# Wumpf/yasph2d

Hardware: AMD Instinct MI355X
Metric: particle-steps/sec (whole node), 2D DFSPH dam-break (higher is better)
Workload: dtype f32

## Files before the change

include/sphx.h:

```cpp
#ifndef SPHX_H
#define SPHX_H

#include <stddef.h>
#include <stdint.h>

#ifdef __cplusplus
extern "C" {
#endif

#define SPHX_ABI_VERSION 5

enum {
    SPHX_OK = 0,
    SPHX_ERR_INVALID_ARGUMENT = 1,
    SPHX_ERR_NO_DEVICE = 2,
    SPHX_ERR_HIP = 3,
    SPHX_ERR_NOT_READY = 4,
    SPHX_ERR_NONFINITE = 5,
    SPHX_ERR_NEIGHBOR_PANIC = 6,
    SPHX_ERR_CAPACITY = 7,
    SPHX_ERR_OUT_OF_DOMAIN = 8
};

enum {
// ... 217 lines not shown
int sphx_gauge_levels(sphx_ctx* ctx, const sphx_gauge* gauges , uint32_t n_gauges, int kernel_kind, int field, float iso,
                      uint32_t flags, sphx_gauge_rec* out , float* values );
int sphx_gauge_reduce(const float* values, const sphx_gauge* gauges, uint32_t n_gauges, float iso, sphx_gauge_rec* out);
int sphx_probe_record(sphx_ctx* ctx, const float* points_xy , uint32_t m_points, const sphx_gauge* gauges ,
                      uint32_t n_gauges, int kernel_kind, int field, float iso, uint32_t max_frames, uint32_t every);
int sphx_probe_get_status(const sphx_ctx* ctx, sphx_probe_status* out);
int sphx_probe_read(sphx_ctx* ctx, uint32_t first_frame, uint32_t n_frames, sphx_probe_rec* points_out ,
                    sphx_gauge_rec* gauges_out , sphx_stats_frame* info );

int sphx_debug_correction_counts(sphx_ctx* ctx, uint64_t out[3]);
int sphx_debug_quiet_counts(sphx_ctx* ctx, uint64_t out[2]);
int sphx_debug_takeover_counts(sphx_ctx* ctx, uint64_t out[3]);

int sphx_debug_rigid_counts(sphx_ctx* ctx, uint64_t out[3]);
int sphx_debug_rigid_predict_counts(sphx_ctx* ctx, uint64_t out[4]);
int sphx_debug_download_accel(sphx_ctx* ctx, float* out_xy);
int sphx_debug_download_wcsph_half_step(sphx_ctx* ctx, float* pos_xy, float* vel_xy, float* density, uint32_t* particle_id);

int sphx_clear_cached(sphx_ctx* ctx);
int sphx_step_begin(sphx_ctx* ctx, float dt_prev, float* out_vmax);
int sphx_step_finish(sphx_ctx* ctx, float dt, sphx_step_stats* out_stats);

typedef struct sphx_timer_law {
    uint32_t adaptive;
    float cfl_factor;
    float particle_diameter;
    uint32_t reserved;
    uint64_t timestep_min_ns;
    uint64_t timestep_max_ns;
    uint64_t simulation_step_ns;
// ... 374 lines not shown
```

yasph2d_amd/__init__.py:

```python
import ctypes as C

import numpy as np

from . import _lib
from ._lib import (FLAG_DENSITY_ITER_CAP, FLAG_DIVERGENCE_ITER_CAP, FLAG_DENSE_CELL, FLAG_NEIGHBOR_CAP, FLAG_STRAY_PARTICLES, FLAG_WARMUP, KERNEL_POLY6,
                   KERNEL_SPIKY, KERNEL_WENDLAND_C2, VISCOSITY_PHYSICAL, VISCOSITY_XSPH, SphxError, SphxKernelTime, SphxParams, SphxStepStats)

__all__ = ["SphxContext", "FluidParticleWorld", "TimeManager", "DFSPHSolver", "DFSPHMultiSolver", "default_params", "duration_from_secs_f32",
           "duration_as_secs_f32", "SphxError", "WCSPHSolver", "VISCOSITY_XSPH", "VISCOSITY_PHYSICAL", "SAMPLE_FIELDS", "gauge_elevation", "contour_chain", "contour_lines", "contour_merge",
           "sample_merge", "query_merge", "render_fit", "render_merge", "track_merge", "track_merge_frames", "write_png", "SCENE_RECT", "TRACK_FIELDS", "MULTI_TRACK_FIELDS", "FIELD_NAMES", "STATS_DTYPE", "STATS_FRAME_DTYPE",
           "GAUGE_DTYPE", "GAUGE_REC_DTYPE", "PROBE_REC_DTYPE", "gauge_reduce"]


def _p(a):
    return a.ctypes.data_as(C.c_void_p) if a is not None else None


LISTS_32BIT = 0xFFFFFFFF


_VISCOSITY_MODELS = {"xsph": VISCOSITY_XSPH, "physical": VISCOSITY_PHYSICAL}


def default_params(smoothing_factor=2.0, particle_density=10000.0, fluid_density=100.0, device=0, fixed_iterations=(0, 0), viscosity="xsph",
# ... 807 lines not shown
        return int(out[0]), int(out[1])

    def takeover_counts(self):
        out = (C.c_uint64 * 3)()
        self._chk(self.L.sphx_debug_takeover_counts(self.h, out))
        return int(out[0]), int(out[1]), int(out[2])

    def rigid_counts(self):
        out = (C.c_uint64 * 3)()
        self._chk(self.L.sphx_debug_rigid_counts(self.h, out))
        return int(out[0]), int(out[1]), int(out[2])

    def rigid_predict_counts(self):
        out = (C.c_uint64 * 4)()
        self._chk(self.L.sphx_debug_rigid_predict_counts(self.h, out))
        return int(out[0]), int(out[1]), int(out[2]), int(out[3])

    def download_accel(self):
        out = np.zeros((self.n, 2), np.float32)
        self._chk(self.L.sphx_debug_download_accel(self.h, out.ctypes.data_as(C.c_void_p)))
        return out

    def download_wcsph_half_step(self):
        n = self.n
        out = dict(pos=np.zeros((n, 2), np.float32), vel=np.zeros((n, 2), np.float32), density=np.zeros(n, np.float32), ids=np.zeros(n, np.uint32))
        self._chk(self.L.sphx_debug_download_wcsph_half_step(self.h, _p(out["pos"]), _p(out["vel"]), _p(out["density"]), _p(out["ids"])))
        return out

    def grid_info(self, which=0):
        out = (C.c_uint32 * 4)()
# ... 695 lines not shown
```

yasph2d_amd/_lib.py:

```python
import ctypes as C
import os
import subprocess

_HERE = os.path.dirname(os.path.abspath(__file__))
LIB_PATH = os.environ.get("SPHX_LIB") or os.path.join(_HERE, "libsphx.so")
CSRC = os.path.join(_HERE, "csrc")

OK, ERR_INVALID_ARGUMENT, ERR_NO_DEVICE, ERR_HIP, ERR_NOT_READY, ERR_NONFINITE, ERR_NEIGHBOR_PANIC, ERR_CAPACITY, ERR_OUT_OF_DOMAIN = range(9)
FLAG_NEIGHBOR_CAP, FLAG_DENSITY_ITER_CAP, FLAG_DIVERGENCE_ITER_CAP, FLAG_WARMUP, FLAG_STRAY_PARTICLES, FLAG_DENSE_CELL = 1, 2, 4, 8, 16, 32
KERNEL_WENDLAND_C2, KERNEL_POLY6, KERNEL_SPIKY = 0, 1, 2
VISCOSITY_XSPH, VISCOSITY_PHYSICAL = 0, 1


class SphxParams(C.Structure):
    _fields_ = [
        ("smoothing_length", C.c_float),
        ("particle_mass", C.c_float),
        ("fluid_density", C.c_float),
        ("particle_radius", C.c_float),
        ("gravity", C.c_float * 2),
        ("grid_min", C.c_float * 2),
        ("xsph_epsilon", C.c_float),
        ("max_avg_density_error", C.c_float),
        ("max_density_iterations", C.c_uint32),
# ... 325 lines not shown
    "sphx_multi_state_load": (_i, [_vp, C.POINTER(_vp), C.POINTER(_u64), _u32, _u32]),
    "sphx_multi_state_digest": (_i, [_vp, C.POINTER(_u64)]),
    "sphx_multi_state_save_file": (_i, [_vp, C.c_char_p]),
    "sphx_multi_state_load_file": (_i, [_vp, C.c_char_p]),
    "sphx_multi_append": (_i, [_vp, _vp, _vp, _u32, C.POINTER(_u32)]),
    "sphx_multi_remove": (_i, [_vp, C.POINTER(SphxRect), _u32, _u32, C.POINTER(_u64)]),
    "sphx_tile_remove_mark": (_i, [_vp, C.POINTER(SphxRect), _u32, _u32]),
    "sphx_tile_remove_fetch": (_i, [_vp, C.POINTER(_u32)]),
    "sphx_tile_append": (_i, [_vp, _vp, _vp, _vp, _u32]),
    "sphx_tile_grow": (_i, [_vp, _u32]),
    "sphx_debug_correction_counts": (_i, [_vp, _vp]),
    "sphx_debug_quiet_counts": (_i, [_vp, _vp]),
    "sphx_debug_takeover_counts": (_i, [_vp, _vp]),
    "sphx_debug_rigid_counts": (_i, [_vp, _vp]),
    "sphx_debug_rigid_predict_counts": (_i, [_vp, _vp]),
    "sphx_debug_download_accel": (_i, [_vp, _vp]),
    "sphx_debug_download_wcsph_half_step": (_i, [_vp, _vp, _vp, _vp, _vp]),
    "sphx_download_by_id": (_i, [_vp, _u32, _u32, _u32, C.POINTER(SphxTrackOut), C.POINTER(_u32)]),
    "sphx_download": (_i, [_vp, _vp, _vp, _vp, _vp]),
    "sphx_download_boundary": (_i, [_vp, _vp, _vp]),
    "sphx_num_particles": (_u32, [_vp]),
    "sphx_num_boundary": (_u32, [_vp]),
    "sphx_sample_points": (_i, [_vp, _vp, _u32, _i, _u32, C.POINTER(SphxSampleOut)]),
    "sphx_sample_grid": (_i, [_vp, _f, _f, _f, _f, _u32, _u32, _i, _u32, C.POINTER(SphxSampleOut)]),
    "sphx_surface_contour": (_i, [_vp, _f, _f, _f, _f, _u32, _u32, _i, _i, _f, _u32, _u32, C.POINTER(SphxContourOut)]),
    "sphx_contour_chain": (_i, [_vp, _u32, _vp, _vp, _vp, C.POINTER(_u32)]),
    "sphx_multi_sample_points": (_i, [_vp, _vp, _u32, _i, _u32, C.POINTER(SphxMultiSampleOut)]),
    "sphx_multi_sample_grid": (_i, [_vp, _f, _f, _f, _f, _u32, _u32, _i, _u32, C.POINTER(SphxMultiSampleOut)]),
    "sphx_sample_merge": (_i, [_u32, C.POINTER(SphxMultiSampleOut), _u32, C.POINTER(SphxMultiSampleOut)]),
    "sphx_multi_query_radius": (_i, [_vp, _vp, _u32, _f, _u64, _u32, C.POINTER(SphxMultiQueryOut)]),
# ... 185 lines not shown
```

yasph2d_amd/csrc/sphx_compute_error_body.inc:

```
    static_assert(!TAKE || KNZ, "the take-over producers are the ones that leave flags");
    constexpr bool SPEC = TAKE && !DIVERGENCE;
    if (la.enabled && la.iter > 1u && scal->loop_done != 0u) return;
    if (dt_dev) dt = *dt_dev;
    if (clear_hist) {
        const uint32_t per = (clear_len + gridDim.x - 1u) / gridDim.x;
        const uint32_t c0 = blockIdx.x * per, c1 = min(c0 + per, clear_len);
        for (uint32_t k = c0 + threadIdx.x; k < c1; k += 256u) clear_hist[k] = 0u;
    }
    __shared__ Stage<2, 0> rec;
    auto put = [&](uint32_t slot, const float4& r) { rec.put_vec01(slot, r); };
    auto take = [&](uint32_t o) { return rec.vec01(o); };
    const uint32_t blk = xcd_bid(K.rev, K.xcd_shift);
    const uint32_t i = blk * 256 + threadIdx.x;
    [[maybe_unused]] bool k_a = false;
    if constexpr (RIGID != 0) {
        static_assert(!DIVERGENCE && PREDICT && KNZ && TAKE, "the rigid form is the density loop's take-over producer with the prediction");
        uint32_t vb = 0;
        if (pa.va.enabled && threadIdx.x < STRIPES) vb = scal->vstripe[threadIdx.x].vmax[pa.va.vslot & 3u];
        const uint32_t verdict = scal->verdict.accel_uniform;
        const float2 v0 = PV.vel[0];
        const uint32_t last = n ? n - 1u : 0u, ic = min(i, last);
        const uint32_t craw = nb.counts[ic];
        const uint32_t wi = (uint32_t)__builtin_amdgcn_readfirstlane(i >> 6);
        const uint32_t ww = wi * 64u < n ? nb.wave[wi] : 0u;
// ... 2 lines not shown
        __shared__ float dt_r;
        if (pa.va.enabled && threadIdx.x < 64) {
            const uint32_t b = wave_max_u32(vb);
            const unsigned long long ns = timer_law_step_ns(pa.law, sqrtf(__uint_as_float(b)));
            const float d = duration_as_secs_f32(ns);
            if (threadIdx.x == 0) dt_r = d;
            if (blockIdx.x == 0) vmax_publish(scal, pa.va, b, pa.law, ns, d);
        }
        if (pa.va.enabled) {
            __syncthreads();
            dt = dt_r;
        }
        k_a = verdict == ta.accel_tag;
        const float4 pvi = make_float4(p_i.x, p_i.y, v0.x + K.ax * dt, v0.y + K.ay * dt);
        const bool finite = ((__float_as_uint(pvi.z) & 0x7f800000u) != 0x7f800000u) && ((__float_as_uint(pvi.w) & 0x7f800000u) != 0x7f800000u);
        DirAhead ahead_r{0xFFFFFFFFu, EMPTY};
        if constexpr (RIGID == 2) {
            if (ta.hist && i < n) {
                uint32_t cx0, cy0;
                cell_of(K, p_i, cx0, cy0);
                ahead_r = dir_ahead(ta.g, cx0, cy0);
            }
        }
        const uint32_t c = i < n ? craw : 0u;
        const bool reaches_static = (c & 0x7fu) != ((c >> 7) & 0x7fu) || (ww >> 31) != 0u;
        const bool walks = __syncthreads_or(reaches_static ? 1 : 0) != 0 || !k_a || !finite || RIGID != 2;
        if (ta.count && threadIdx.x == 0) {
            Stripe& s = scal->stripe[blockIdx.x % STRIPES];
            if (k_a && blk * 256u < n) atomicAdd(walks ? &s.rp_walk : &s.rp_exit, 1u);
            if (!k_a && blockIdx.x == 0) atomicAdd(&s.rp_noverdict, 1u);
// ... 121 lines not shown
```

yasph2d_amd/csrc/sphx_correct_body.inc:

```
    static_assert(!ZS || (!WARM && !TILE), "the skip belongs to the plain corrections");
    static_assert(!QF || ZS, "the decide-first form falls back to the skip's decision");
    float dt = WARM ? ca.dt : (la.enabled ? la.dt : ca.dt);
    if (dt_dev) {
        dt = *dt_dev;
        inv_dt = 1.0f / dt;
    }
    constexpr bool RES = !WARM;
    const bool need_verdict = RES && ra.enabled && (THIN ? vblk == 0u : blockIdx.x == 0);
    const bool judge = need_verdict && threadIdx.x < 64;
    unsigned long long hi = 0, lo = 0, snap_h = 0, snap_l = 0;
    uint32_t sticky = 0;
    uint32_t jmark = ~ra.rseq;
    const uint32_t rp = ra.rseq & 1u;
    if (RES && ra.enabled) {
        const uint32_t done_before = (la.enabled && la.iter > 1u) ? scal->loop_done : 0u;
        if (judge) {
            residual_stripe_load(scal, hi, lo);
            if constexpr (ZS)
                if (threadIdx.x < STRIPES) jmark = scal->mstripe[threadIdx.x].knz_mark;
            snap_h = scal->snap_hi[rp ^ 1u];
            snap_l = scal->snap_lo[rp ^ 1u];
            sticky = scal->flags;
        }
        if (done_before != 0u && done_before < la.iter) {
// ... 111 lines not shown
            __syncthreads();
            if constexpr (THIN && INV_DT) {
                if (!quiet_s && ca.hist && vblk == 0u && threadIdx.x == 0) scal->spec.flags = 0u;
            }
            if (quiet_s) {
                if (zs.count && threadIdx.x == 0) {
                    unsigned long long stands_for = 1ull;
                    if constexpr (THIN) {
                        stands_for = 0ull;
                        for (uint32_t v = vblk; v < vgrid; v += gridDim.x) stands_for += xcd_map(v, vgrid, K.rev, K.xcd_shift) * 256u < n ? 1ull : 0ull;
                    }
                    atomicAdd(&scal->stripe[blockIdx.x % STRIPES].zs_skipped, stands_for);
                    atomicAdd(&scal->stripe[blockIdx.x % STRIPES].zs_quiet, stands_for);
                }
                if constexpr (THIN && INV_DT) {
                    if (ca.hist && vblk == 0u && threadIdx.x == 0) {
                        const uint32_t f = scal->spec.flags;
                        if (f) {
                            atomicOr(&scal->flags, f);
                            scal->spec.flags = 0u;
                        }
                    }
                }
                verdict();
                if constexpr (THIN) SPHX_CORRECT_LEAVE(true);
                float2 pnew = make_float2(0.0f, 0.0f);
                DirAhead ahead{0xFFFFFFFFu, EMPTY};
                if (i < n) {
                    if (INV_DT) {
                        if (ca.hist) {
// ... 180 lines not shown
```

yasph2d_amd/csrc/sphx_handoff.hpp:

```cpp
#pragma once
#include <cstdint>
#include <cstring>

namespace sphx {

struct BuildHandoff {
    enum Kind : uint8_t { None, WarmApplied, FirstErrors };
    Kind kind = None;
    bool has_flags = false, warm_taken = false;
    uint32_t mark_tag = 0;
    struct Taken {
        bool fused, flags_usable, warm_taken;
    };
    static BuildHandoff warm_applied() { return BuildHandoff{WarmApplied, false, false, 0u}; }
    static BuildHandoff first_errors(bool flags, uint32_t tag, bool taken) { return BuildHandoff{FirstErrors, flags, flags && taken, tag}; }
    void clear() { *this = BuildHandoff{}; }
    bool first_errors_pending() const { return kind == FirstErrors; }
    bool take_warm() {
        const bool applied = kind == WarmApplied;
        if (applied) clear();
        return applied;
    }
    Taken take_first_errors(bool first_divergence, uint32_t rseq) {
        if (kind != FirstErrors || !first_divergence) return Taken{false, false, false};
// ... 76 lines not shown
    void filled() { *this = AccelUniform{}; }
    Taken read() {
        const Taken t{owed, false, tag};
        owed = false;
        return t;
    }
    Taken take(bool substitute) {
        const bool k_a = substitute && uniform;
        const Taken t{owed && !k_a, k_a, tag};
        if (t.fill) owed = false;
        uniform = false;
        return t;
    }
};

}
```

yasph2d_amd/csrc/sphx_internal.hpp:

```cpp
#pragma once
#include <hip/hip_runtime.h>

#include <dlfcn.h>

#include <algorithm>
#include <cstdint>
#include <cstdlib>
#include <cstdio>
#include <cstring>
#include <functional>
#include <map>
#include <string>
#include <vector>

#include "../../include/sphx.h"
#include "sphx_handoff.hpp"

namespace sphx {

constexpr uint32_t EMPTY = 0xFFFFFFFFu;
constexpr uint32_t MAX_NEIGHBORS = 64;
constexpr uint32_t BLOCK_SHIFT = 6;
constexpr uint32_t BLOCK_CELLS = 4096;
constexpr uint32_t SCAN_TILE = 4096;
// ... 109 lines not shown
    uint32_t knz_mark;
    uint32_t vmix_mark;
    uint32_t pad[30];
};
static_assert(sizeof(MarkStripe) == 128, "one stripe, one cache line");
struct alignas(128) SpecLine {
    uint32_t flags;
    uint32_t pad0;
    unsigned long long moved;
    uint32_t pad[28];
};
struct alignas(128) VerdictLine {
    uint32_t accel_uniform;
    uint32_t pad[31];
};
struct DevScalars {
    uint32_t flags;
    uint32_t ticket;
    uint32_t sort_total;
    float dt;
    uint32_t loop_done;
    uint32_t pad0;
    unsigned long long snap_hi[2], snap_lo[2];
    uint32_t rigid_exits, rigid_marked;
    uint32_t pad[16];
    Stripe stripe[STRIPES];
    VmaxStripe vstripe[STRIPES];
    MarkStripe mstripe[STRIPES];
    SpecLine spec;
    VerdictLine verdict;
};

struct Mailbox {
    volatile uint32_t seq;
    uint32_t flags;
    uint32_t vmax_sq_bits;
    uint32_t quiet_seq;
    double err_sum;
    unsigned long long nb_entries;
    unsigned long long owned_cum;
    unsigned long long rem_entries;
    uint32_t sort_total;
    uint32_t dt_bits;
    unsigned long long dt_ns;
    volatile uint32_t loop_gen_done;
// ... 185 lines not shown
    uint32_t thin_grid = 0;
    int quiet_takeover_density = 1;
    bool take_over(bool divergence) const {
        return !tile_mode && (divergence || quiet_takeover_density) && (quiet_takeover == 2 || (quiet_takeover == 1 && quiet_hint[divergence ? 1 : 0]));
    }
    unsigned long long thin_launches = 0, takeover_producers = 0;
    int rigid_skip = -1;
    bool rigid_on() const { return !tile_mode && (rigid_skip < 0 ? N >= 4000000u : rigid_skip != 0); }
    sphx::VelMarks velmarks;
    uint32_t gather_seq = 0;
    bool rigid_hint = false;
    uint32_t rigid_judged = 0;
    void rigid_forget() {
        velmarks.wrote();
        accel_uniform.velocities_written();
        rigid_hint = false;
        rigid_judged = 0;
    }
    unsigned long long rigid_launches = 0;
    int rigid_predict = 2;
    sphx::AccelUniform accel_uniform;
    unsigned long long rigid_predict_launches = 0;
    float2* accel = nullptr;
    float *density = nullptr, *alpha = nullptr, *alpha2 = nullptr, *kappa = nullptr, *stiff = nullptr;
    float *kappa2 = nullptr, *stiff2 = nullptr;
    uint32_t *pid = nullptr, *pid2 = nullptr;
    uint32_t *key = nullptr, *order = nullptr;
    uint32_t idx_cap = 0;
    uint32_t soff() const { return capN; }
    float2 *bpos = nullptr, *bpos2 = nullptr;
    uint32_t *bid = nullptr, *bid2 = nullptr;
    sphx::Grid gdyn, gstat;
    bool have_fluid_bbox = false;
    uint32_t fb[4] = {0, 0, 0, 0};
    uint32_t builds_since_cover = 0;
    bool need_expand = false;
    bool need_recover = false;
// ... 97 lines not shown
```

yasph2d_amd/csrc/sphx_kernels.hip:

```cpp
#include "sphx_internal.hpp"
#include "sphx_sqrt.hpp"
#include "sphx_xcd.hpp"

namespace sphx {

__device__ __forceinline__ uint32_t part1by1(uint32_t x) {
    x &= 0xffffu;
    x = (x ^ (x << 8)) & 0x00ff00ffu;
    x = (x ^ (x << 4)) & 0x0f0f0f0fu;
    x = (x ^ (x << 2)) & 0x33333333u;
    x = (x ^ (x << 1)) & 0x55555555u;
    return x;
}
__device__ __forceinline__ uint32_t morton2(uint32_t x, uint32_t y) { return (part1by1(y) << 1) | part1by1(x); }

__device__ __forceinline__ uint32_t spread6(uint32_t v) {
    v &= 63u;
    v = (v | (v << 4)) & 0x30Fu;
    v = (v | (v << 2)) & 0x333u;
    v = (v | (v << 1)) & 0x555u;
    return v;
}
__device__ __forceinline__ uint32_t sat_u16(float v) {
    v = fminf(fmaxf(v, 0.0f), 65535.0f);
// ... 584 lines not shown
    float* r2_out;
    const float* r3_in;
    float* r3_out;
    const uint32_t* u_in;
    uint32_t* u_out;
    DevScalars* count_owned;
    DevScalars* flags;
    float advect_dt;
    uint32_t advect_below;
    uint32_t fix_owner;
    float cell_inv, gmin_x, gmin_y;
    TileRect own;
    uint32_t rank_by_id;
    uint32_t nt_cold;
    uint32_t vmix_tag;
};
#ifndef SPHX_GATHER_PER_LANE
#define SPHX_GATHER_PER_LANE 1
#endif
constexpr uint32_t GATHER_PER_LANE = SPHX_GATHER_PER_LANE;
__global__ __launch_bounds__(256) void k_rank_gather(const uint32_t* __restrict__ order, const uint32_t* __restrict__ cidx, uint32_t n,
                                                      uint32_t n_in, const uint2* __restrict__ fine, GatherArgs a,
                                                      const uint32_t* __restrict__ n_dev, uint32_t rev) {
    if (n_dev) n = min(n, *n_dev);
    const uint32_t b0 = xcd_bid(xcd_packed_rev(rev), xcd_packed_shift(rev)) * (256u * GATHER_PER_LANE);
    if (b0 >= n) return;
    uint2 vref = make_uint2(0u, 0u);
    if (a.vmix_tag) vref = *(const uint2*)a.vel_in;
    bool vmix = false;
    constexpr int RANK_L = 5, RANK_R = 6;
    constexpr uint32_t ORD_HALO = 8, SPAN = 256u * GATHER_PER_LANE;
    static_assert(RANK_L <= (int)ORD_HALO && RANK_R <= (int)ORD_HALO, "window of order[] words in LDS");
    __shared__ uint32_t sord[SPAN + 2 * ORD_HALO];
    uint32_t own[GATHER_PER_LANE];
#pragma unroll
    for (uint32_t u = 0; u < GATHER_PER_LANE; ++u) {
        own[u] = order[min(b0 + u * 256u + threadIdx.x, n - 1u)];
        sord[ORD_HALO + u * 256u + threadIdx.x] = own[u];
    }
    if (threadIdx.x < 2 * ORD_HALO) {
        const int32_t k = threadIdx.x < ORD_HALO ? (int32_t)(b0 + threadIdx.x) - (int32_t)ORD_HALO : (int32_t)(b0 + SPAN + threadIdx.x - ORD_HALO);
        sord[threadIdx.x < ORD_HALO ? threadIdx.x : SPAN + threadIdx.x] = order[(uint32_t)min(max(k, 0), (int32_t)n - 1)];
    }
    bool ok[GATHER_PER_LANE];
    float2 q[GATHER_PER_LANE], v[GATHER_PER_LANE];
    float r1[GATHER_PER_LANE], r2[GATHER_PER_LANE], r3[GATHER_PER_LANE];
    uint32_t id[GATHER_PER_LANE];
#pragma unroll
    for (uint32_t u = 0; u < GATHER_PER_LANE; ++u) {
        const uint32_t i = own[u] & ORDER_INDEX;
        ok[u] = b0 + u * 256u + threadIdx.x < n && i < n_in;
        const uint32_t ic = ok[u] ? i : 0u;
        q[u] = a.pos_in[ic];
        v[u] = a.vel_in ? a.vel_in[ic] : make_float2(0.0f, 0.0f);
        r1[u] = a.r_in ? a.r_in[ic] : 0.0f, r2[u] = a.r2_in ? a.r2_in[ic] : 0.0f, r3[u] = a.r3_in ? a.r3_in[ic] : 0.0f;
        id[u] = a.u_in ? a.u_in[ic] : 0u;
    }
    __syncthreads();
#pragma unroll
    for (uint32_t u = 0; u < GATHER_PER_LANE; ++u) {
        if (!ok[u]) continue;
        const uint32_t p = b0 + u * 256u + threadIdx.x, i = own[u] & ORDER_INDEX;
        uint32_t near[RANK_L + RANK_R + 1];
#pragma unroll
        for (int d = -RANK_L; d <= RANK_R; ++d) near[d + RANK_L] = sord[(int)(ORD_HALO + u * 256u + threadIdx.x) + d];
        uint32_t heads_l = 0, heads_r = 0;
#pragma unroll
        for (int d = 0; d <= RANK_L; ++d) heads_l |= (near[RANK_L - d] >> 31) << d;
#pragma unroll
// ... 56 lines not shown
        if (a.r3_in) a.r3_out[dst] = r3[u];
        if (a.u_in) {
            uint32_t idd = id[u];
            if (a.fix_owner && i < a.advect_below) {
                const uint32_t cx = sat_u16((qd.x - a.gmin_x) * a.cell_inv), cy = sat_u16((qd.y - a.gmin_y) * a.cell_inv);
                if (!rect_has(a.own, cx, cy, 0u)) idd &= 0x7FFFFFFFu;
            }
            store_cold(&a.u_out[dst], idd, a.nt_cold);
            if (a.count_owned) {
                const unsigned long long m = __ballot((idd >> 31) != 0);
                if (m && (threadIdx.x & 63) == (uint32_t)(__ffsll((long long)__ballot(1)) - 1))
                    atomicAdd(&a.count_owned->stripe[blockIdx.x % STRIPES].owned, (unsigned long long)__popcll(m));
            }
        }
    }
    if (a.vmix_tag) {
        const bool ref_bad = (vref.x & 0x7f800000u) == 0x7f800000u || (vref.y & 0x7f800000u) == 0x7f800000u;
        const unsigned long long m = __ballot(vmix || ref_bad);
        if (m && (threadIdx.x & 63) == (uint32_t)(__ffsll((long long)__ballot(1)) - 1)) a.flags->mstripe[blockIdx.x % STRIPES].vmix_mark = a.vmix_tag;
    }
}

__global__ __launch_bounds__(256) void k_iota(uint32_t* __restrict__ a, uint32_t n) {
    const uint32_t i = blockIdx.x * 256 + threadIdx.x;
    if (i < n) a[i] = i;
}
__global__ __launch_bounds__(256) void k_fill_f32(float* __restrict__ a, uint32_t from, uint32_t n, float v) {
    const uint32_t i = from + blockIdx.x * 256 + threadIdx.x;
    if (i < n) a[i] = v;
}
// ... 1369 lines not shown
template <bool DIVERGENCE, bool PREDICT = false, bool KNZ = false, bool TAKE = false>
__global__ TRAV_BOUNDS void k_compute_error(PVr PV, const float* __restrict__ density,
                                                        const float* __restrict__ alpha, uint32_t n, uint32_t soff, Consts K, float dt,
                                                        NbView nb, float* __restrict__ kbuf, float* __restrict__ warm_zero,
                                                        DevScalars* __restrict__ scal, const float* __restrict__ dt_dev, LoopArgs la,
                                                        uint32_t* __restrict__ clear_hist, uint32_t clear_len, PredArgs pa,
                                                        uint32_t* __restrict__ knz, uint32_t knz_tag,
                                                        std::conditional_t<TAKE && !DIVERGENCE, CountArgs, NoTake> ta) {
    constexpr int RIGID = 0;
#include "sphx_compute_error_body.inc"
}

struct RigidTake : CountArgs {
    uint32_t accel_tag;
    uint32_t count;
};
template <bool EXIT>
__global__ TRAV_BOUNDS void k_compute_error_rigid(PVr PV, const float* __restrict__ density,
                                                              const float* __restrict__ alpha, uint32_t n, uint32_t soff, Consts K, float dt,
                                                              NbView nb, float* __restrict__ kbuf, float* __restrict__ warm_zero,
                                                              DevScalars* __restrict__ scal, const float* __restrict__ dt_dev, LoopArgs la,
                                                              uint32_t* __restrict__ clear_hist, uint32_t clear_len, PredArgs pa,
                                                              uint32_t* __restrict__ knz, uint32_t knz_tag, RigidTake ta) {
    constexpr bool DIVERGENCE = false, PREDICT = true, KNZ = true, TAKE = true;
    constexpr int RIGID = EXIT ? 2 : 1;
#include "sphx_compute_error_body.inc"
}

__global__ __launch_bounds__(256) void k_accel_materialize(float2* __restrict__ accel, uint32_t n, uint32_t vgrid, float ax, float ay,
                                                           const DevScalars* __restrict__ scal, uint32_t tag) {
// ... 132 lines not shown
```

yasph2d_amd/csrc/sphx_launch.inc:

```
#include <algorithm>
#include <cmath>

using namespace sphx;

static std::string g_create_error;

#define SPHX_HIP(ctx, expr)                                                        \
    do {                                                                           \
        hipError_t e__ = (expr);                                                   \
        if (e__ != hipSuccess) return (ctx)->fail(SPHX_ERR_HIP, #expr, hipGetErrorString(e__)); \
    } while (0)

namespace {

inline uint32_t nblocks(uint32_t n, uint32_t per = 256) {
    const uint32_t b = (n + per - 1) / per;
    return per == 256 ? (b + 7u) & ~7u : b;
}
inline double kbar_of(const sphx_ctx* c) { return (c->N && c->nb_last) ? (double)c->nb_last / (double)c->N : 12.0; }
inline double list_bytes(const sphx_ctx* c) {
    if (!c->K.remote_cap) return 2.0 + 4.0 * kbar_of(c);
    const double rbar = c->N ? (double)c->rem_last / (double)c->N : 0.5;
    return 2.0 + 4.0 / 64.0 + (4.0 / 3.0) * kbar_of(c) + 4.0 * rbar + 4.0 / 256.0;
}
// ... 492 lines not shown
    c->ahead.valid = false;
    flush_pending_advect(c);
}

int build_grid(sphx_ctx* c, Grid& g, const float2* pos, uint32_t n, const GatherArgs& ga, float advect_dt, bool ring, uint32_t* tile_n = nullptr,
               bool mark_velocities = false) {
    hipStream_t st = c->stream;
    DevScalars* ds = c->d_scal;
    const uint32_t len = g.len();
    const uint32_t nt = nblocks(len, c->scan_two_pass ? SCAN_TILE : SCAN1_TILE);
    const bool counted = &g == &c->gdyn && advect_dt > 0 && !tile_n && c->pending.is_for(n);
    const bool partial = &g == &c->gdyn && tile_n && advect_dt == 0.0f && !counted && c->pending.is_for_first_of(n);
    const uint32_t first = partial ? c->pending.n() : 0u;
    if (&g == &c->gdyn) c->velmarks.wrote();
    if (&g == &c->gdyn) c->accel_uniform.velocities_written();
    if (counted || partial)
        c->pending.forget();
    else
        drop_fused_count(c);
    if (n > first && !counted) {
        const uint32_t gbc = std::max(1u, nblocks(n - first));
        if (advect_dt > 0)
            launch(c, "advect+cell_count", (16.0 + 4 + 4) * n, [&] {
                hipLaunchKernelGGL(k_key_count<true>, dim3(gbc), dim3(256), 0, st, c->pv(), (const float2*)nullptr, n, advect_dt, c->K,
                                   g.view(), g.hist, c->key, ring ? 1u : 0u, ds, first);
            });
        else
            launch(c, "cell_count", (8.0 + 4 + 4) * (n - first), [&] {
                hipLaunchKernelGGL(k_key_count<false>, dim3(gbc), dim3(256), 0, st, PVr{nullptr, nullptr}, pos, n, 0.0f, c->K, g.view(),
                                   g.hist, c->key, ring ? 1u : 0u, ds, first);
// ... 30 lines not shown
                *tile_n = seq;
            }
        }
        const uint32_t gb2 = std::max(8u, (nblocks(ng, 256 * GATHER_PER_LANE) + 7u) & ~7u);
        double gbytes = 4;
        gbytes += ga.vel_in ? (16 + 16) : 16;
        if (ga.r_in) gbytes += 8;
        if (ga.r2_in) gbytes += 8;
        if (ga.r3_in) gbytes += 8;
        if (ga.u_in) gbytes += 8;
        GatherArgs gm = ga;
        if (mark_velocities && &g == &c->gdyn && !tile_n && ga.vel_in) {
            if (++c->gather_seq == 0) c->gather_seq = 1;
            gm.vmix_tag = c->gather_seq;
        }
        if (ng)
            launch(c, "gather_attributes", gbytes * ng, [&] {
                hipLaunchKernelGGL(k_rank_gather, dim3(gb2), dim3(256), 0, st, (const uint32_t*)c->order, (const uint32_t*)c->key, ng, n,
                                   (const uint2*)g.fine, gm, tile_n ? (const uint32_t*)&ds->sort_total : (const uint32_t*)nullptr, xcd_pack(c->K.rev, xcd_shift_of(c)));
            });
        if (ng && gm.vmix_tag) c->velmarks.made(gm.vmix_tag);
    }
    return SPHX_OK;
}

int ensure_index_scratch(sphx_ctx* c) {
    const uint32_t need = std::max(std::max(std::max(c->N, c->capN), c->B), 1u);
    if (need <= c->idx_cap) return SPHX_OK;
    int rc;
    if ((rc = dev_alloc(c, &c->key, need))) return rc;
// ... 225 lines not shown
    if (c->N) {
        const uint32_t n = c->N;
        auto go = [&](auto kernel, const DivArgs& dv) {
            hipLaunchKernelGGL(kernel, dim3(nblocks(n)), dim3(256), 0, st, (const float2*)c->posA, n, c->soff(), c->K, c->gdyn.nview(), c->gstat.nview(),
                               c->nb_list, c->nb_counts, c->nb_wave, c->nb_remote, c->density, c->alpha, c->d_scal, n_dev, dv);
        };
        c->handoff.clear();
        if (fuse && fuse_warm) {
            DivArgs dv{};
            dv.velw = c->vel;
            dv.warm = c->stiff;
            dv.lim = -0.5f * c->K.rho0 * c->K.rho0;
            launch(c, "neighbor_build+density_alpha+divergence_warmstart", (8.0 + list_bytes(c) + 8.0 + 8.0 + 8.0 + 4.0) * n, [&] { go(k_neighbor_build<3>, dv); });
            c->handoff = BuildHandoff::warm_applied();
            c->velmarks.wrote();
            c->accel_uniform.velocities_written();
        } else if (fuse && fuse_div) {
            DivArgs dv{};
            dv.vel = (const float2*)c->vel;
            dv.kbuf = c->kbuf;
            dv.knz = zero_skip_flags(c);
            dv.knz_tag = c->res_seq + 1u;
            const bool take = take_div;
            if (take) {
                dv.warm = c->stiff;
                c->takeover_producers += 1;
            }
            launch(c, "neighbor_build+density_alpha+density_change", (8.0 + list_bytes(c) + 8.0 + 8.0 + 4.0) * n,
                   [&] { take ? go(k_neighbor_build<2, true>, dv) : go(k_neighbor_build<2>, dv); });
            c->handoff = BuildHandoff::first_errors(dv.knz != nullptr, dv.knz_tag, take);
// ... 90 lines not shown
    dev_free(&old_kappa);
    dev_free(&old_stiff);
    dev_free(&old_alpha);
    dev_free(&old_accel);
    dev_free(&old_pid);
    c->capN = cap;
    return SPHX_OK;
}

inline bool device_loop(const sphx_ctx* c) { return !c->tile_mode && !c->host_loop; }


void launch_predict(sphx_ctx* c, const char* label, float dt, const VmaxArgs& va = VmaxArgs{}, const TimerLaw& tl = TimerLaw{}) {
    const uint32_t n = c->N;
    c->velmarks.wrote();
    take_accel(c, false);
    launch(c, label, 24.0 * n, [&] { hipLaunchKernelGGL(k_predict, dim3(nblocks(n)), dim3(256), 0, c->stream, c->vel, (const float2*)c->accel, n, dt, c->d_scal, va, tl); });
}

void launch_compute_error(sphx_ctx* c, bool divergence, float dt, const float* dt_dev, const LoopArgs& la, uint32_t* clear_hist, uint32_t clear_len,
                          const PredArgs* pred, uint32_t* knz, uint32_t knz_tag, bool take_warm = false,
                          const CountArgs& take_count = CountArgs{}) {
    const uint32_t n = c->N;
    const double lb = list_bytes(c);
    if (pred) c->velmarks.wrote();
    auto go = [&](auto kernel, float* warm, const PredArgs& pa, auto take) {
        hipLaunchKernelGGL(kernel, dim3(nblocks(n)), dim3(256), 0, c->stream, c->pv(), (const float*)c->density, (const float*)c->alpha, n, c->soff(), c->K, dt,
                           c->nbv(), c->kbuf, warm, c->d_scal, dt_dev, la, clear_hist, clear_len, pa, knz, knz_tag, take);
    };
    if (divergence) {
        launch(c, "compute_density_change", (16 + 4 + 4 + lb) * n, [&] {
            if (knz && take_warm) return go(k_compute_error<true, false, true, true>, c->stiff, PredArgs{}, NoTake{});
            if (knz) return go(k_compute_error<true, false, true>, nullptr, PredArgs{}, NoTake{});
            go(k_compute_error<true>, nullptr, PredArgs{}, NoTake{});
        });
    } else if (pred) {
        PredArgs pa = *pred;
        pa.accel = c->accel;
        pa.vel_out = c->vel2;
        const AccelUniform::Taken au = take_accel(c, c->rigid_predict != 0 && knz && take_warm && c->K.q_noclamp && !c->tile_mode);
        if (au.k_a) {
            c->rigid_predict_launches += 1;
            const RigidTake rt{take_count, au.tag, c->zero_skip_count ? 1u : 0u};
            auto go_rigid = [&](auto kernel) {
                hipLaunchKernelGGL(kernel, dim3(nblocks(n)), dim3(256), 0, c->stream, c->pv(), (const float*)c->density, (const float*)c->alpha, n, c->soff(), c->K, dt,
                                   c->nbv(), c->kbuf, c->kappa, c->d_scal, dt_dev, la, clear_hist, clear_len, pa, knz, knz_tag, rt);
            };
            const double bytes = c->rigid_predict == 2 ? (8 + 4 + 4 + 2 + 4 + 8 + 4 + 4 + 8) * (double)n : (16 + 8 + 4 + 4 + 4 + lb) * n;
            return launch(c, "velocity_prediction+compute_density_error", bytes,
                          [&] { c->rigid_predict == 2 ? go_rigid(k_compute_error_rigid<true>) : go_rigid(k_compute_error_rigid<false>); });
        }
        launch(c, "velocity_prediction+compute_density_error", (16 + 8 + 8 + 4 + 4 + 4 + lb) * n, [&] {
            if (knz && take_warm) return go(k_compute_error<false, true, true, true>, c->kappa, pa, take_count);
            if (knz) return go(k_compute_error<false, true, true>, nullptr, pa, NoTake{});
            go(k_compute_error<false, true>, nullptr, pa, NoTake{});
        });
    } else {
        launch(c, "compute_density_error", (16 + 4 + 4 + 4 + lb) * n + (clear_hist ? 4.0 * clear_len : 0.0), [&] {
// ... 9 lines not shown
    return knz && c->K.q_noclamp && !tc.pid && std::isfinite(c->K.mass) && c->K.mass > 0.0f && (dt_dev || divergence || (inv_dt > 0.0f && std::isfinite(inv_dt)));
}
void launch_correct(sphx_ctx* c, bool divergence, float dt, const float* dt_dev, const CountArgs& ca, const LoopArgs& la, const ResArgs& ra, bool first,
                    const TileClassArgs& tc, const uint32_t* knz, bool warm_taken = false) {
    const uint32_t n = c->N, f = first ? 1u : 0u;
    const float inv_dt = 1.0f / dt, lim = -0.5f * c->K.rho0 * c->K.rho0;
    const char* const label = divergence ? "correct_velocity_with_divergence_error" : "correct_velocity_with_density_error";
    float* warm = divergence ? c->stiff : c->kappa;
    const bool skip_ok = correct_skip_ok(c, divergence, dt, dt_dev, tc, knz);
    const ZeroSkipArgs zs{skip_ok ? knz : nullptr, c->zero_skip_count ? 1u : 0u};
    const bool quiet_first = zs.knz && c->quiet_hint[divergence ? 1 : 0];
    const bool thin = first && warm_taken && zs.knz && (divergence || ca.hist);
    if ((quiet_first || thin) && c->zero_skip_count) c->qf_launches += 1;
    thin ? c->velmarks.thin(ra.rseq) : c->velmarks.wrote();
    c->accel_uniform.velocities_written();
    if (thin) {
        c->thin_launches += 1;
        const uint32_t vblocks = nblocks(n);
        auto go_thin = [&](auto kernel) {
            hipLaunchKernelGGL(kernel, dim3(std::min(vblocks, c->thin_grid ? c->thin_grid : 2048u)), dim3(256), 0, c->stream, c->vel, (const float2*)c->posA,
                               (const float*)c->kbuf, warm, n, c->soff(), c->K, inv_dt, lim, c->nbv(), dt_dev, ca, c->d_scal, la, ra, zs, vblocks);
        };
        const double bytes = (16 + 8 + 12 + 8 + list_bytes(c) + (ca.hist ? 8 : 0)) * n;
        return launch(c, label, bytes, [&] { divergence ? go_thin(k_correct_thin<false>) : go_thin(k_correct_thin<true>); }, false);
    }
    auto go = [&](auto kernel, const ZeroSkipArgs& zsa) {
        hipLaunchKernelGGL(kernel, dim3(nblocks(n)), dim3(256), 0, c->stream, c->vel, (const float2*)c->posA, (const float*)c->kbuf, warm, n, c->soff(), c->K, inv_dt,
                           lim, c->nbv(), dt_dev, ca, c->d_scal, la, ra, f, tc, zsa);
    };
    launch(c, label, (16 + 8 + 12 + 8 + list_bytes(c) + (ca.hist ? (tc.pid ? 8 + 4 : 8) : 0)) * n, [&] {
        if (divergence && quiet_first) return go(k_correct<false, false, false, true, true>, zs);
        if (quiet_first) return go(k_correct<false, true, false, true, true>, zs);
        if (divergence && zs.knz) return go(k_correct<false, false, false, true>, zs);
        if (divergence) return go(k_correct<false, false>, zs);
        if (tc.pid) return go(k_correct<false, true, true>, ZeroSkipArgs{});
        if (zs.knz) return go(k_correct<false, true, false, true>, zs);
        go(k_correct<false, true>, zs);
    });
}

void launch_warmstart(sphx_ctx* c, bool divergence, float dt, const float* dt_dev, bool labelled) {
    const uint32_t n = c->N;
    c->velmarks.wrote();
    c->accel_uniform.velocities_written();
    const float inv_dt = 1.0f / dt, lim = -0.5f * c->K.rho0 * c->K.rho0;
    auto one = [&](auto kernel, float* warm) {
        hipLaunchKernelGGL(kernel, dim3(nblocks(n)), dim3(256), 0, c->stream, c->vel, (const float2*)c->posA, (const float*)c->kbuf, warm, n, c->soff(), c->K, inv_dt,
                           lim, c->nbv(), dt_dev, CountArgs{}, c->d_scal, LoopArgs{}, ResArgs{}, 0u, TileClassArgs{}, ZeroSkipArgs{});
    };
    auto go = [&] { divergence ? one(k_correct<true, false>, c->stiff) : one(k_correct<true, true>, c->kappa); };
    if (!labelled) return go();
    launch(c, divergence ? "correct_divergence_error_warmstart" : "correct_density_error_warmstart", (16 + 8 + 8 + 4 + list_bytes(c)) * n, go);
}

struct IterSpec {
    bool divergence, first;
    float dt;
    const float* dt_dev = nullptr;
    uint32_t* out_warm = nullptr;
// ... 316 lines not shown
    if (!c || !out) return SPHX_ERR_INVALID_ARGUMENT;
    SPHX_HIP(c, hipSetDevice(c->device));
    SPHX_HIP(c, hipStreamSynchronize(c->stream));
    std::vector<Stripe> st(STRIPES);
    SPHX_HIP(c, hipMemcpy(st.data(), c->d_scal->stripe, sizeof(Stripe) * STRIPES, hipMemcpyDeviceToHost));
    out[0] = c->rigid_predict_launches;
    out[1] = out[2] = out[3] = 0;
    for (const Stripe& s : st) {
        out[1] += s.rp_exit;
        out[2] += s.rp_walk;
        out[3] += s.rp_noverdict;
    }
    return SPHX_OK;
}

int sphx_debug_download_accel(sphx_ctx* c, float* out_xy) {
    if (!c || (c->N && !out_xy)) return SPHX_ERR_INVALID_ARGUMENT;
    SPHX_HIP(c, hipSetDevice(c->device));
    read_accel(c);
    SPHX_HIP(c, hipStreamSynchronize(c->stream));
    if (c->N) SPHX_HIP(c, hipMemcpy(out_xy, c->accel, (size_t)c->N * 8, hipMemcpyDeviceToHost));
    return SPHX_OK;
}

int sphx_debug_quiet_counts(sphx_ctx* c, uint64_t out[2]) {
    if (!c || !out) return SPHX_ERR_INVALID_ARGUMENT;
    SPHX_HIP(c, hipSetDevice(c->device));
    SPHX_HIP(c, hipStreamSynchronize(c->stream));
    std::vector<Stripe> st(STRIPES);
    SPHX_HIP(c, hipMemcpy(st.data(), c->d_scal->stripe, sizeof(Stripe) * STRIPES, hipMemcpyDeviceToHost));
// ... 29 lines not shown
    if (const char* e = std::getenv("SPHX_HOST_LOOP")) c->host_loop = e[0] == '1';
    if (const char* e = std::getenv("SPHX_RUN_AHEAD")) c->run_ahead = e[0] != '0';
    if (const char* e = std::getenv("SPHX_FUSE_PREDICT")) c->fuse_predict = e[0] != '0';
    if (const char* e = std::getenv("SPHX_LAZY_TABLE")) c->lazy_table = e[0] != '0' ? 1 : 0;
    if (const char* e = std::getenv("SPHX_STREAM_LISTS")) c->stream_lists = e[0] != '0' ? 1 : 0;
    if (const char* e = std::getenv("SPHX_NT_COLD_STORES")) c->nt_cold_stores = e[0] != '0' ? 1 : 0;
    if (const char* e = std::getenv("SPHX_TILE_FUSE_CLASS")) c->tile_fuse_class = e[0] != '0';
    if (const char* e = std::getenv("SPHX_FUSE_DIV")) c->fuse_div = e[0] != '0';
    if (const char* e = std::getenv("SPHX_XCD_CHUNK")) c->xcd_chunk = (int)xcd_shift_clamp(std::atoi(e));
    if (const char* e = std::getenv("SPHX_ALTERNATE_SWEEP")) c->alternate_sweep = e[0] == '2' ? 2 : (e[0] != '0');
    if (const char* e = std::getenv("SPHX_ZERO_SKIP")) c->zero_skip = e[0] != '0';
    if (const char* e = std::getenv("SPHX_ZERO_SKIP_COUNT")) c->zero_skip_count = e[0] == '1';
    if (const char* e = std::getenv("SPHX_QUIET_TAKEOVER")) c->quiet_takeover = std::strcmp(e, "force") == 0 ? 2 : (e[0] != '0' ? 1 : 0);
    if (const char* e = std::getenv("SPHX_QUIET_TAKEOVER_DENSITY")) c->quiet_takeover_density = e[0] != '0';
    if (const char* e = std::getenv("SPHX_RIGID_SKIP")) c->rigid_skip = std::strcmp(e, "force") == 0 ? 2 : (e[0] != '0' ? 1 : 0);
    if (const char* e = std::getenv("SPHX_RIGID_PREDICT")) c->rigid_predict = std::strcmp(e, "accel") == 0 ? 1 : (e[0] != '0' ? 2 : 0);
    if (const char* e = std::getenv("SPHX_THIN_GRID")) c->thin_grid = (uint32_t)std::max(0, std::atoi(e));
    if (const char* e = std::getenv("SPHX_FUSE_WARM")) c->fuse_warm = e[0] != '0';
    c->P = *params;
    c->device = params->device;
    const float h = params->smoothing_length;
    const float PI_F = (float)3.14159265358979323846;
    Consts& K = c->K;
    K.h = h;
    K.radius_sq = h * h;
    K.cell_inv = 1.0f / h;
    K.gmin_x = params->grid_min[0];
    K.gmin_y = params->grid_min[1];
    K.w_hinv = 1.0f / h;
    K.w_norm = 4.0f * 7.0f / (PI_F * rs_powi(h, 2));
// ... 1154 lines not shown
```

Baseline: 13.84 billion.

## Publish uniform rigid velocity and skip per-particle velocity reads in gather

When the rigid predict path finds every particle shares the same accelerated velocity, the compute-error kernel publishes that velocity plus a tag to a device cache line. A host-side VelStar state machine tracks whether a matching thin correction confirmed it and no other velocity write happened since. The next rank gather then reads a single broadcast velocity instead of scattered per-particle loads. This saves 8 bytes per particle of gather traffic but adds a tag handshake, invalidation calls at every velocity writer, and a correctness risk if the uniformity check is wrong.

```diff
diff --git a/include/sphx.h b/include/sphx.h
--- a/include/sphx.h
+++ b/include/sphx.h
@@ -255,6 +255,7 @@
 
 int sphx_debug_rigid_counts(sphx_ctx* ctx, uint64_t out[3]);
 int sphx_debug_rigid_predict_counts(sphx_ctx* ctx, uint64_t out[4]);
+int sphx_debug_rigid_velocity_counts(sphx_ctx* ctx, uint64_t out[4]);
 int sphx_debug_download_accel(sphx_ctx* ctx, float* out_xy);
 int sphx_debug_download_wcsph_half_step(sphx_ctx* ctx, float* pos_xy, float* vel_xy, float* density, uint32_t* particle_id);
 
diff --git a/yasph2d_amd/__init__.py b/yasph2d_amd/__init__.py
--- a/yasph2d_amd/__init__.py
+++ b/yasph2d_amd/__init__.py
@@ -845,6 +845,11 @@
     def rigid_predict_counts(self):
         out = (C.c_uint64 * 4)()
         self._chk(self.L.sphx_debug_rigid_predict_counts(self.h, out))
+        return int(out[0]), int(out[1]), int(out[2]), int(out[3])
+
+    def rigid_velocity_counts(self):
+        out = (C.c_uint64 * 4)()
+        self._chk(self.L.sphx_debug_rigid_velocity_counts(self.h, out))
         return int(out[0]), int(out[1]), int(out[2]), int(out[3])
 
     def download_accel(self):
diff --git a/yasph2d_amd/_lib.py b/yasph2d_amd/_lib.py
--- a/yasph2d_amd/_lib.py
+++ b/yasph2d_amd/_lib.py
@@ -363,6 +363,7 @@
     "sphx_debug_takeover_counts": (_i, [_vp, _vp]),
     "sphx_debug_rigid_counts": (_i, [_vp, _vp]),
     "sphx_debug_rigid_predict_counts": (_i, [_vp, _vp]),
+    "sphx_debug_rigid_velocity_counts": (_i, [_vp, _vp]),
     "sphx_debug_download_accel": (_i, [_vp, _vp]),
     "sphx_debug_download_wcsph_half_step": (_i, [_vp, _vp, _vp, _vp, _vp]),
     "sphx_download_by_id": (_i, [_vp, _u32, _u32, _u32, C.POINTER(SphxTrackOut), C.POINTER(_u32)]),
diff --git a/yasph2d_amd/csrc/sphx_compute_error_body.inc b/yasph2d_amd/csrc/sphx_compute_error_body.inc
--- a/yasph2d_amd/csrc/sphx_compute_error_body.inc
+++ b/yasph2d_amd/csrc/sphx_compute_error_body.inc
@@ -40,6 +40,14 @@
         k_a = verdict == ta.accel_tag;
         const float4 pvi = make_float4(p_i.x, p_i.y, v0.x + K.ax * dt, v0.y + K.ay * dt);
         const bool finite = ((__float_as_uint(pvi.z) & 0x7f800000u) != 0x7f800000u) && ((__float_as_uint(pvi.w) & 0x7f800000u) != 0x7f800000u);
+        if (ta.vel_tag && blockIdx.x == 0 && threadIdx.x == 0) {
+            VelStarLine& w = scal->vstar;
+            w.tag = ta.vel_tag;
+            w.uniform = (k_a && finite) ? 1u : 0u;
+            w.vx = pvi.z;
+            w.vy = pvi.w;
+            w.published += (k_a && finite) ? 1u : 0u;
+        }
         DirAhead ahead_r{0xFFFFFFFFu, EMPTY};
         if constexpr (RIGID == 2) {
             if (ta.hist && i < n) {
diff --git a/yasph2d_amd/csrc/sphx_correct_body.inc b/yasph2d_amd/csrc/sphx_correct_body.inc
--- a/yasph2d_amd/csrc/sphx_correct_body.inc
+++ b/yasph2d_amd/csrc/sphx_correct_body.inc
@@ -149,6 +149,7 @@
                     atomicAdd(&scal->stripe[blockIdx.x % STRIPES].zs_quiet, stands_for);
                 }
                 if constexpr (THIN && INV_DT) {
+                    if (vblk == 0u && threadIdx.x == 0) scal->vstar.confirm = ra.rseq;
                     if (ca.hist && vblk == 0u && threadIdx.x == 0) {
                         const uint32_t f = scal->spec.flags;
                         if (f) {
diff --git a/yasph2d_amd/csrc/sphx_handoff.hpp b/yasph2d_amd/csrc/sphx_handoff.hpp
--- a/yasph2d_amd/csrc/sphx_handoff.hpp
+++ b/yasph2d_amd/csrc/sphx_handoff.hpp
@@ -114,4 +114,21 @@
     }
 };
 
+struct VelStar {
+    bool live = false, thin_seen = false;
+    uint32_t tag = 0, n = 0;
+    void made(uint32_t rseq, uint32_t count) { *this = rseq ? VelStar{true, false, rseq, count} : VelStar{}; }
+    void thin(uint32_t rseq) {
+        if (!live) return;
+        if (thin_seen || rseq != tag) return wrote();
+        thin_seen = true;
+    }
+    void wrote() { *this = VelStar{}; }
+    uint32_t take(uint32_t count) {
+        const uint32_t t = (live && thin_seen && count == n) ? tag : 0u;
+        wrote();
+        return t;
+    }
+};
+
 }
diff --git a/yasph2d_amd/csrc/sphx_internal.hpp b/yasph2d_amd/csrc/sphx_internal.hpp
--- a/yasph2d_amd/csrc/sphx_internal.hpp
+++ b/yasph2d_amd/csrc/sphx_internal.hpp
@@ -147,6 +147,13 @@
     uint32_t accel_uniform;
     uint32_t pad[31];
 };
+struct alignas(128) VelStarLine {
+    uint32_t tag, uniform, confirm, pad0;
+    float vx, vy;
+    uint32_t published, substituted;
+    uint32_t pad[24];
+};
+static_assert(sizeof(VelStarLine) == 128, "one cache line");
 struct DevScalars {
     uint32_t flags;
     uint32_t ticket;
@@ -162,6 +169,7 @@
     MarkStripe mstripe[STRIPES];
     SpecLine spec;
     VerdictLine verdict;
+    VelStarLine vstar;
 };
 
 struct Mailbox {
@@ -377,6 +385,7 @@
     void rigid_forget() {
         velmarks.wrote();
         accel_uniform.velocities_written();
+        velstar.wrote();
         rigid_hint = false;
         rigid_judged = 0;
     }
@@ -384,6 +393,9 @@
     int rigid_predict = 2;
     sphx::AccelUniform accel_uniform;
     unsigned long long rigid_predict_launches = 0;
+    int rigid_vel = 1;
+    sphx::VelStar velstar;
+    unsigned long long velstar_producers = 0, velstar_gathers = 0;
     float2* accel = nullptr;
     float *density = nullptr, *alpha = nullptr, *alpha2 = nullptr, *kappa = nullptr, *stiff = nullptr;
     float *kappa2 = nullptr, *stiff2 = nullptr;
diff --git a/yasph2d_amd/csrc/sphx_kernels.hip b/yasph2d_amd/csrc/sphx_kernels.hip
--- a/yasph2d_amd/csrc/sphx_kernels.hip
+++ b/yasph2d_amd/csrc/sphx_kernels.hip
@@ -622,6 +622,7 @@
     uint32_t rank_by_id;
     uint32_t nt_cold;
     uint32_t vmix_tag;
+    uint32_t vstar_tag;
 };
 #ifndef SPHX_GATHER_PER_LANE
 #define SPHX_GATHER_PER_LANE 1
@@ -636,6 +637,8 @@
     uint2 vref = make_uint2(0u, 0u);
     if (a.vmix_tag) vref = *(const uint2*)a.vel_in;
     bool vmix = false;
+    const uint4 vw = *(const uint4*)&a.flags->vstar.tag;
+    const bool vsub = (a.vstar_tag != 0u) & (vw.x == a.vstar_tag) & (vw.z == a.vstar_tag) & (vw.y != 0u);
     constexpr int RANK_L = 5, RANK_R = 6;
     constexpr uint32_t ORD_HALO = 8, SPAN = 256u * GATHER_PER_LANE;
     static_assert(RANK_L <= (int)ORD_HALO && RANK_R <= (int)ORD_HALO, "window of order[] words in LDS");
@@ -660,7 +663,7 @@
         ok[u] = b0 + u * 256u + threadIdx.x < n && i < n_in;
         const uint32_t ic = ok[u] ? i : 0u;
         q[u] = a.pos_in[ic];
-        v[u] = a.vel_in ? a.vel_in[ic] : make_float2(0.0f, 0.0f);
+        v[u] = a.vel_in ? a.vel_in[vsub ? 0u : ic] : make_float2(0.0f, 0.0f);
         r1[u] = a.r_in ? a.r_in[ic] : 0.0f, r2[u] = a.r2_in ? a.r2_in[ic] : 0.0f, r3[u] = a.r3_in ? a.r3_in[ic] : 0.0f;
         id[u] = a.u_in ? a.u_in[ic] : 0u;
     }
@@ -747,6 +750,7 @@
             }
         }
     }
+    if (vsub && b0 == 0u && threadIdx.x == 0) a.flags->vstar.substituted += 1u;
     if (a.vmix_tag) {
         const bool ref_bad = (vref.x & 0x7f800000u) == 0x7f800000u || (vref.y & 0x7f800000u) == 0x7f800000u;
         const unsigned long long m = __ballot(vmix || ref_bad);
@@ -2146,6 +2150,7 @@
 struct RigidTake : CountArgs {
     uint32_t accel_tag;
     uint32_t count;
+    uint32_t vel_tag;
 };
 template <bool EXIT>
 __global__ TRAV_BOUNDS void k_compute_error_rigid(PVr PV, const float* __restrict__ density,
diff --git a/yasph2d_amd/csrc/sphx_launch.inc b/yasph2d_amd/csrc/sphx_launch.inc
--- a/yasph2d_amd/csrc/sphx_launch.inc
+++ b/yasph2d_amd/csrc/sphx_launch.inc
@@ -530,6 +530,7 @@
     const uint32_t first = partial ? c->pending.n() : 0u;
     if (&g == &c->gdyn) c->velmarks.wrote();
     if (&g == &c->gdyn) c->accel_uniform.velocities_written();
+    const uint32_t vstar_tag = &g == &c->gdyn ? c->velstar.take(n) : 0u;
     if (counted || partial)
         c->pending.forget();
     else
@@ -590,6 +591,11 @@
             if (++c->gather_seq == 0) c->gather_seq = 1;
             gm.vmix_tag = c->gather_seq;
         }
+        if (vstar_tag && counted && !tile_n && ga.vel_in && ga.advect_below == 0xFFFFFFFFu) {
+            gm.vstar_tag = vstar_tag;
+            gbytes -= 8;
+            c->velstar_gathers += 1;
+        }
         if (ng)
             launch(c, "gather_attributes", gbytes * ng, [&] {
                 hipLaunchKernelGGL(k_rank_gather, dim3(gb2), dim3(256), 0, st, (const uint32_t*)c->order, (const uint32_t*)c->key, ng, n,
@@ -845,6 +851,7 @@
             launch(c, "neighbor_build+density_alpha+divergence_warmstart", (8.0 + list_bytes(c) + 8.0 + 8.0 + 8.0 + 4.0) * n, [&] { go(k_neighbor_build<3>, dv); });
             c->handoff = BuildHandoff::warm_applied();
             c->velmarks.wrote();
+            c->velstar.wrote();
             c->accel_uniform.velocities_written();
         } else if (fuse && fuse_div) {
             DivArgs dv{};
@@ -965,6 +972,7 @@
 void launch_predict(sphx_ctx* c, const char* label, float dt, const VmaxArgs& va = VmaxArgs{}, const TimerLaw& tl = TimerLaw{}) {
     const uint32_t n = c->N;
     c->velmarks.wrote();
+    c->velstar.wrote();
     take_accel(c, false);
     launch(c, label, 24.0 * n, [&] { hipLaunchKernelGGL(k_predict, dim3(nblocks(n)), dim3(256), 0, c->stream, c->vel, (const float2*)c->accel, n, dt, c->d_scal, va, tl); });
 }
@@ -975,6 +983,7 @@
     const uint32_t n = c->N;
     const double lb = list_bytes(c);
     if (pred) c->velmarks.wrote();
+    c->velstar.wrote();
     auto go = [&](auto kernel, float* warm, const PredArgs& pa, auto take) {
         hipLaunchKernelGGL(kernel, dim3(nblocks(n)), dim3(256), 0, c->stream, c->pv(), (const float*)c->density, (const float*)c->alpha, n, c->soff(), c->K, dt,
                            c->nbv(), c->kbuf, warm, c->d_scal, dt_dev, la, clear_hist, clear_len, pa, knz, knz_tag, take);
@@ -992,7 +1001,10 @@
         const AccelUniform::Taken au = take_accel(c, c->rigid_predict != 0 && knz && take_warm && c->K.q_noclamp && !c->tile_mode);
         if (au.k_a) {
             c->rigid_predict_launches += 1;
-            const RigidTake rt{take_count, au.tag, c->zero_skip_count ? 1u : 0u};
+            const uint32_t vel_tag = c->rigid_vel && take_count.hist ? knz_tag : 0u;
+            c->velstar.made(vel_tag, n);
+            if (vel_tag) c->velstar_producers += 1;
+            const RigidTake rt{take_count, au.tag, c->zero_skip_count ? 1u : 0u, vel_tag};
             auto go_rigid = [&](auto kernel) {
                 hipLaunchKernelGGL(kernel, dim3(nblocks(n)), dim3(256), 0, c->stream, c->pv(), (const float*)c->density, (const float*)c->alpha, n, c->soff(), c->K, dt,
                                    c->nbv(), c->kbuf, c->kappa, c->d_scal, dt_dev, la, clear_hist, clear_len, pa, knz, knz_tag, rt);
@@ -1032,6 +1044,7 @@
     if ((quiet_first || thin) && c->zero_skip_count) c->qf_launches += 1;
     thin ? c->velmarks.thin(ra.rseq) : c->velmarks.wrote();
     c->accel_uniform.velocities_written();
+    thin && !divergence ? c->velstar.thin(ra.rseq) : c->velstar.wrote();
     if (thin) {
         c->thin_launches += 1;
         const uint32_t vblocks = nblocks(n);
@@ -1061,6 +1074,7 @@
     const uint32_t n = c->N;
     c->velmarks.wrote();
     c->accel_uniform.velocities_written();
+    c->velstar.wrote();
     const float inv_dt = 1.0f / dt, lim = -0.5f * c->K.rho0 * c->K.rho0;
     auto one = [&](auto kernel, float* warm) {
         hipLaunchKernelGGL(kernel, dim3(nblocks(n)), dim3(256), 0, c->stream, c->vel, (const float2*)c->posA, (const float*)c->kbuf, warm, n, c->soff(), c->K, inv_dt,
@@ -1407,6 +1421,19 @@
     return SPHX_OK;
 }
 
+int sphx_debug_rigid_velocity_counts(sphx_ctx* c, uint64_t out[4]) {
+    if (!c || !out) return SPHX_ERR_INVALID_ARGUMENT;
+    SPHX_HIP(c, hipSetDevice(c->device));
+    SPHX_HIP(c, hipStreamSynchronize(c->stream));
+    uint32_t dev[2] = {0u, 0u};
+    SPHX_HIP(c, hipMemcpy(dev, &c->d_scal->vstar.published, sizeof(dev), hipMemcpyDeviceToHost));
+    out[0] = c->velstar_producers;
+    out[1] = dev[0];
+    out[2] = c->velstar_gathers;
+    out[3] = dev[1];
+    return SPHX_OK;
+}
+
 int sphx_debug_download_accel(sphx_ctx* c, float* out_xy) {
     if (!c || (c->N && !out_xy)) return SPHX_ERR_INVALID_ARGUMENT;
     SPHX_HIP(c, hipSetDevice(c->device));
@@ -1466,6 +1493,7 @@
     if (const char* e = std::getenv("SPHX_QUIET_TAKEOVER")) c->quiet_takeover = std::strcmp(e, "force") == 0 ? 2 : (e[0] != '0' ? 1 : 0);
     if (const char* e = std::getenv("SPHX_QUIET_TAKEOVER_DENSITY")) c->quiet_takeover_density = e[0] != '0';
     if (const char* e = std::getenv("SPHX_RIGID_SKIP")) c->rigid_skip = std::strcmp(e, "force") == 0 ? 2 : (e[0] != '0' ? 1 : 0);
+    if (const char* e = std::getenv("SPHX_RIGID_VEL")) c->rigid_vel = e[0] != '0' ? 1 : 0;
     if (const char* e = std::getenv("SPHX_RIGID_PREDICT")) c->rigid_predict = std::strcmp(e, "accel") == 0 ? 1 : (e[0] != '0' ? 2 : 0);
     if (const char* e = std::getenv("SPHX_THIN_GRID")) c->thin_grid = (uint32_t)std::max(0, std::atoi(e));
     if (const char* e = std::getenv("SPHX_FUSE_WARM")) c->fuse_warm = e[0] != '0';
```

After: 13.77 billion. No clear change (-0.5%).
